# mistralai/mistral-inference

Hardware: NVIDIA H100
Metric: decode tokens/sec (bf16, batch=1, seq=4k) [+ prefill TFLOPS, both vs roofline] (higher is better)
Workload: dtype bf16

## Files before the change

include/mistral_b200.h:

```cpp
#ifndef MISTRAL_B200_H_
#define MISTRAL_B200_H_

#include <stddef.h>
#include <stdint.h>

#ifdef __cplusplus
extern "C" {
#endif

#define MB200_ABI_VERSION 1

#define MB200_OK 0
#define MB200_E_INVALID (-1)
#define MB200_E_WORKSPACE (-2)
#define MB200_E_CUDA (-3)

int mb200_abi_version(void);
const char* mb200_last_error(void);
int mb200_device_info(int* sm_count, int* max_smem_optin);

int mb200_rmsnorm(const void* x, const void* w, void* out, int64_t T, int64_t dim, float eps, void* stream);

int mb200_attn_qkv(const void* x, const void* norm_w, const void* wqkv, const float* rope, const int32_t* positions,
                   void* q_out, void* k_out, void* v_out, void* cache_k, void* cache_v, const int32_t* cache_rows,
// ... 26 lines not shown
int mb200_argmax_rows(const float* logits, int64_t* out_dev, int64_t T, int64_t vocab, void* stream);
int mb200_logprob_gather(const float* logits, const int64_t* target_dev, float* out_dev, int64_t T, int64_t vocab, void* stream);
int mb200_sample_top_p(const float* logits, const float* uniform_dev, int64_t* out_dev, int64_t T, int64_t vocab,
                       float temperature, float top_p, void* stream);

typedef struct mb200_moe_comm {
  int32_t n_ranks, my_rank;
  void* peer_yw[8];
  void* my_flags;
  void* peer_flags[8];
  void* epoch;
  void* done_counter;
} mb200_moe_comm;
int mb200_moe_sizes(int64_t T, int64_t n_experts, int64_t top_k, int64_t* tile_rows, int64_t* rows_cap, int64_t* plan_words);
int mb200_moe_route(const void* hn, const void* gate_w, int64_t T, int64_t dim, int64_t n_experts, int64_t top_k, int64_t shard_rank,
                    int64_t shard_world, int32_t* sel, void* wts, int32_t* slot, int32_t* plan, void* xs, void* row_w, void* stream);
int mb200_moe_grouped_ffn(const void* xs, const void* const* w13_host, const void* const* w2_host, const int32_t* plan, const void* row_w,
                          const int32_t* slot, const void* residual, void* g, void* yw, void* out, int64_t T, int64_t dim,
                          int64_t hidden, int64_t n_experts, int64_t top_k, const mb200_moe_comm* comm, void* workspace,
                          size_t workspace_bytes, void* stream);

int mb200_comm_alloc(size_t bytes, void** ptr_out);
int mb200_comm_free(void* ptr);
int mb200_comm_export(void* ptr, void* handle_out64);
int mb200_comm_open(const void* handle64, void** ptr_out);
int mb200_comm_close(void* ptr);

size_t mb200_workspace_bytes(int64_t T, int64_t dim, int64_t n_heads, int64_t n_kv_heads, int64_t head_dim,
                             int64_t hidden, int64_t vocab, int64_t max_batch);

typedef struct mb200_layer_desc {
  const void* wqkv;
  const void* wo;
  const void* w13;
  const void* w2;
  const void* attn_norm;
  const void* ffn_norm;
  void* cache_k;
  void* cache_v;
} mb200_layer_desc;

int mb200_decode_step(const mb200_layer_desc* layers_dev, const int32_t* windows_dev, int64_t n_layers, const void* emb,
                      const void* final_norm, const void* w_out, const float* rope, const int64_t* token_dev, int64_t pos,
                      int64_t batch_row, float* logits, int64_t* next_token_dev, int64_t dim, int64_t hidden, int64_t n_heads, int64_t n_kv_heads,
                      int64_t head_dim, int64_t vocab, float eps, int64_t n_experts, int64_t top_k, const void* const* moe_gate_dev,
                      const void* const* moe_w13_dev, const void* const* moe_w2_dev, void* workspace, size_t workspace_bytes, void* stream);

#define MB200_SKINNY_MAX_T 4

#define MB200_WORKSPACE_HEADER_BYTES (64 * 1024)

int mb200_debug_set_decode_timeline(void* device_buffer);
int mb200_debug_set_barrier_timeline(void* device_buffer);
int mb200_debug_launch_log(int enable, char* out, size_t out_bytes);

int mb200_test_gemm_naive(const void* a, const void* w, float* c, int64_t T, int64_t N, int64_t K, void* stream);

#ifdef __cplusplus
}
#endif
#endif
```

mistral_inference_b200/_abi.py:

```python
import ctypes
import os
from ctypes import c_char_p, c_float, c_int, c_int64, c_size_t, c_void_p
from pathlib import Path
from typing import Optional

import torch

_LIB_PATH = Path(os.environ.get("MB200_LIB_PATH") or Path(__file__).resolve().parent / "libmb200.so")
_lib: Optional[ctypes.CDLL] = None

ABI_VERSION = 1
SKINNY_MAX_T = 4
WORKSPACE_HEADER_BYTES = 64 * 1024

_SIGNATURES = {
    "mb200_abi_version": (c_int, []),
    "mb200_last_error": (c_char_p, []),
    "mb200_device_info": (c_int, [ctypes.POINTER(c_int), ctypes.POINTER(c_int)]),
    "mb200_rmsnorm": (c_int, [c_void_p, c_void_p, c_void_p, c_int64, c_int64, c_float, c_void_p]),
    "mb200_attn_qkv": (c_int, [c_void_p, c_void_p, c_void_p, c_void_p, c_void_p, c_void_p, c_void_p, c_void_p, c_void_p, c_void_p,
                               c_void_p, c_int64, c_int64, c_int64, c_int64, c_int64, c_float, c_void_p, c_size_t, c_void_p]),
    "mb200_kv_ring_write": (c_int, [c_void_p, c_void_p, c_void_p, c_void_p, c_void_p, c_int64, c_int64, c_int64, c_void_p]),
    "mb200_attn_decode": (c_int, [c_void_p, c_void_p, c_void_p, c_void_p, c_void_p, c_int64, c_int64, c_int64, c_int64, c_int64,
                                  c_int64, c_void_p, c_size_t, c_void_p]),
    "mb200_attn_prefill": (c_int, [c_void_p, c_void_p, c_void_p, c_void_p, c_void_p, c_void_p, c_void_p, c_void_p, c_int64, c_int64,
                                   c_int64, c_int64, c_int64, c_int64, c_int64, c_int, c_void_p]),
    "mb200_linear_residual": (c_int, [c_void_p, c_void_p, c_void_p, c_void_p, c_int64, c_int64, c_int64, c_void_p, c_size_t, c_void_p]),
    "mb200_ffn_gateup": (c_int, [c_void_p, c_void_p, c_void_p, c_void_p, c_int64, c_int64, c_int64, c_float, c_void_p, c_size_t,
                                 c_void_p]),
    "mb200_lm_head": (c_int, [c_void_p, c_void_p, c_void_p, c_void_p, c_int64, c_int64, c_int64, c_float, c_void_p, c_size_t,
                              c_void_p]),
    "mb200_decode_meta": (c_int, [c_void_p, c_void_p, c_int64, c_void_p, c_int64, c_void_p]),
    "mb200_argmax_rows": (c_int, [c_void_p, c_void_p, c_int64, c_int64, c_void_p]),
    "mb200_logprob_gather": (c_int, [c_void_p, c_void_p, c_void_p, c_int64, c_int64, c_void_p]),
    "mb200_sample_top_p": (c_int, [c_void_p, c_void_p, c_void_p, c_int64, c_int64, c_float, c_float, c_void_p]),
    "mb200_moe_sizes": (c_int, [c_int64, c_int64, c_int64, ctypes.POINTER(c_int64), ctypes.POINTER(c_int64), ctypes.POINTER(c_int64)]),
    "mb200_moe_route": (c_int, [c_void_p, c_void_p, c_int64, c_int64, c_int64, c_int64, c_int64, c_int64, c_void_p, c_void_p, c_void_p, c_void_p,
                                c_void_p, c_void_p, c_void_p]),
    "mb200_moe_grouped_ffn": (c_int, [c_void_p, c_void_p, c_void_p, c_void_p, c_void_p, c_void_p, c_void_p, c_void_p, c_void_p, c_void_p, c_int64,
                                      c_int64, c_int64, c_int64, c_int64, c_void_p, c_void_p, c_size_t, c_void_p]),
    "mb200_comm_alloc": (c_int, [c_size_t, ctypes.POINTER(c_void_p)]),
    "mb200_comm_free": (c_int, [c_void_p]),
    "mb200_comm_export": (c_int, [c_void_p, c_void_p]),
    "mb200_comm_open": (c_int, [c_void_p, ctypes.POINTER(c_void_p)]),
    "mb200_comm_close": (c_int, [c_void_p]),
    "mb200_workspace_bytes": (c_size_t, [c_int64] * 8),
    "mb200_decode_step": (c_int, [c_void_p, c_void_p, c_int64, c_void_p, c_void_p, c_void_p, c_void_p, c_void_p, c_int64, c_int64,
                                  c_void_p, c_void_p, c_int64, c_int64, c_int64, c_int64, c_int64, c_int64, c_float, c_int64, c_int64, c_void_p,
                                  c_void_p, c_void_p, c_void_p, c_size_t, c_void_p]),
    "mb200_debug_set_decode_timeline": (c_int, [c_void_p]),
    "mb200_debug_set_barrier_timeline": (c_int, [c_void_p]),
    "mb200_debug_launch_log": (c_int, [c_int, c_void_p, c_size_t]),
    "mb200_test_gemm_naive": (c_int, [c_void_p, c_void_p, c_void_p, c_int64, c_int64, c_int64, c_void_p]),
}


class Mb200Error(RuntimeError):
    pass


def library_path() -> Path:
    return _LIB_PATH


def lib() -> ctypes.CDLL:
    global _lib
    if _lib is not None:
        return _lib
    if not _LIB_PATH.exists():
        raise Mb200Error(
            f"{_LIB_PATH} not found: build it with `python -m mistral_inference_b200.build` "
            "(there is no PyTorch/CPU fallback for the hot path)")
    handle = ctypes.CDLL(str(_LIB_PATH), mode=os.RTLD_LOCAL if hasattr(os, "RTLD_LOCAL") else 0)
    for name, (restype, argtypes) in _SIGNATURES.items():
        fn = getattr(handle, name)
        fn.restype = restype
        fn.argtypes = argtypes
    if handle.mb200_abi_version() != ABI_VERSION:
        raise Mb200Error(f"libmb200 ABI {handle.mb200_abi_version()} != expected {ABI_VERSION}")
    _lib = handle
    return handle


def _check(rc: int, what: str) -> None:
    if rc != 0:
        msg = lib().mb200_last_error()
        raise Mb200Error(f"{what} failed ({rc}): {msg.decode() if msg else '?'}")


def _ptr(t: Optional[torch.Tensor]) -> Optional[int]:
    if t is None:
        return None
    assert t.is_cuda and t.is_contiguous(), "libmb200 takes contiguous CUDA tensors"
    return t.data_ptr()


def _stream() -> int:
    return torch.cuda.current_stream().cuda_stream


class Workspace:

    def __init__(self, nbytes: int, device: torch.device):
        self.buf = torch.zeros(max(int(nbytes), WORKSPACE_HEADER_BYTES + 256), dtype=torch.uint8, device=device)
# ... 148 lines not shown


def comm_alloc(nbytes: int) -> int:
    p = c_void_p(0)
    _check(lib().mb200_comm_alloc(nbytes, ctypes.byref(p)), "mb200_comm_alloc")
    return int(p.value)


def comm_free(ptr: int) -> None:
    _check(lib().mb200_comm_free(ptr), "mb200_comm_free")


def comm_export(ptr: int) -> bytes:
    h = ctypes.create_string_buffer(64)
    _check(lib().mb200_comm_export(ptr, ctypes.cast(h, c_void_p)), "mb200_comm_export")
    return h.raw


def comm_open(handle: bytes) -> int:
    h = ctypes.create_string_buffer(handle, 64)
    p = c_void_p(0)
    _check(lib().mb200_comm_open(ctypes.cast(h, c_void_p), ctypes.byref(p)), "mb200_comm_open")
    return int(p.value)


def comm_close(ptr: int) -> None:
    _check(lib().mb200_comm_close(ptr), "mb200_comm_close")


def decode_meta(seqpos_dev: torch.Tensor, meta_dev: torch.Tensor, windows) -> None:
    B = seqpos_dev.shape[0]
    arr = (ctypes.c_int32 * len(windows))(*[int(w) for w in windows])
    assert seqpos_dev.dtype == torch.int32 and meta_dev.dtype == torch.int32 and meta_dev.numel() >= 3 * B + 1 + 2 * B * len(windows)
    _check(lib().mb200_decode_meta(_ptr(seqpos_dev), _ptr(meta_dev), B, ctypes.cast(arr, c_void_p), len(windows), _stream()), "mb200_decode_meta")


def decode_step(layers_dev, windows_dev, n_layers, emb, final_norm, w_out, rope, token_dev, pos, batch_row, logits, next_token, dim, hidden,
                n_heads, n_kv_heads, head_dim, vocab, eps, ws: Workspace, n_experts: int = 0, top_k: int = 0, moe_gate=None, moe_w13=None,
                moe_w2=None) -> None:
    _check(lib().mb200_decode_step(_ptr(layers_dev), _ptr(windows_dev), n_layers, _ptr(emb), _ptr(final_norm), _ptr(w_out), _ptr(rope),
                                   _ptr(token_dev), pos, batch_row, _ptr(logits), _ptr(next_token), dim, hidden, n_heads, n_kv_heads, head_dim,
                                   vocab, eps, n_experts, top_k, _ptr(moe_gate), _ptr(moe_w13), _ptr(moe_w2), ws.ptr, ws.nbytes, _stream()),
           "mb200_decode_step")


def set_decode_timeline(buf: Optional[torch.Tensor]) -> None:
    _check(lib().mb200_debug_set_decode_timeline(_ptr(buf)), "mb200_debug_set_decode_timeline")


def set_barrier_timeline(buf: Optional[torch.Tensor]) -> None:
    _check(lib().mb200_debug_set_barrier_timeline(_ptr(buf)), "mb200_debug_set_barrier_timeline")


def launch_log(enable: bool) -> list:
    buf = ctypes.create_string_buffer(32768)
    _check(lib().mb200_debug_launch_log(int(enable), ctypes.cast(buf, c_void_p), len(buf)), "mb200_debug_launch_log")
    return buf.value.decode().splitlines()


def test_gemm_naive(a, w) -> torch.Tensor:
    T, K = a.shape
    c = torch.empty(T, w.shape[0], dtype=torch.float32, device=a.device)
    _check(lib().mb200_test_gemm_naive(_ptr(a), _ptr(w), _ptr(c), T, w.shape[0], K, _stream()), "mb200_test_gemm_naive")
    return c
```

mistral_inference_b200/csrc/abi.cu:

```cuda
#include <cmath>
#include <cstdlib>
#include <cstring>

#include "attn_decode.cuh"
#include "attn_decode_tma.cuh"
#include "attn_prefill.cuh"
#include "attn_prefill_wgmma.cuh"
#include "decode_megakernel.cuh"
#include "elementwise.cuh"
#include "gemm_mma.cuh"
#include "gemm_streamk.cuh"
#include "gemm_wgmma.cuh"
#include "moe.cuh"
#include "sampling.cuh"
#include "skinny_linear.cuh"

namespace mb200 {
thread_local char g_err[512] = "";
thread_local bool g_launch_log_on = false;
thread_local bool g_launch_log_overflow = false;
thread_local size_t g_launch_log_len = 0;
thread_local char g_launch_log[kLaunchLogBytes] = "";
static unsigned long long* g_mk_prof = nullptr;
static unsigned long long* g_mk_prof_bar = nullptr;

constexpr size_t kWsHeader = 64 * 1024;
inline size_t align256(size_t v) { return (v + 255) & ~(size_t)255; }

static int run_rmsnorm(const void* x, const void* w, void* out, int64_t T, int64_t dim, float eps, cudaStream_t st) {
  MB_CHECK_ARG(dim % 8 == 0 && T >= 0, "rmsnorm: dim=%lld must be a multiple of 8", (long long)dim);
  if (T == 0) return MB200_OK;
  MB_CHECK_CUDA(launch_pdl(rmsnorm_kernel, dim3((unsigned)T), dim3(256), 0, st, (const uint4*)x, (const uint4*)w, (uint4*)out, (int)dim, eps));
  return MB200_OK;
}

template <int MODE>
static int run_linear(const void* x, const void* norm_w, const void* w, const EpiParams& epi, int64_t T, int64_t N, int64_t K, float eps,
                      void* workspace, size_t workspace_bytes, cudaStream_t st) {
  MB_CHECK_ARG(T >= 1, "linear: T=%lld", (long long)T);
  if (T <= MB200_SKINNY_MAX_T) {
    SkinnyParams p;
    p.x = x;
    p.norm_w = norm_w;
    p.w = w;
    p.N = (int)N;
    p.K = (int)K;
    p.eps = eps;
    p.epi = epi;
    return norm_w ? launch_skinny<MODE, true>(p, (int)T, st) : launch_skinny<MODE, false>(p, (int)T, st);
  }
  const void* a = x;
  if (norm_w) {
    const size_t need = kWsHeader + SK_PARTIAL_BYTES + align256((size_t)T * K * 2);
    if (workspace == nullptr || workspace_bytes < need) return fail(MB200_E_WORKSPACE, "linear: workspace %zu < %zu", workspace_bytes, need);
    void* normed = (uint8_t*)workspace + kWsHeader + SK_PARTIAL_BYTES;
    int rc = run_rmsnorm(x, norm_w, normed, T, K, eps, st);
    if (rc) return rc;
    a = normed;
  }
  GemmParams g;
  g.a = a;
  g.w = w;
  g.T = (int)T;
  g.N = (int)N;
  g.K = (int)K;
  g.epi = epi;
  if (streamk_eligible(T, N, K)) return launch_streamk<MODE>(g, workspace, workspace_bytes, kWsHeader, st);
  if (wgmma_gemm_eligible(T, N, K)) return launch_gemm_wgmma<MODE>(g, st);
  return launch_gemm_mma<MODE>(g, st);
}
}

using namespace mb200;

extern "C" {

int mb200_abi_version(void) { return MB200_ABI_VERSION; }
// ... 383 lines not shown
  auto cut_ok = [](int64_t K) { const int64_t nch = (K + MK_MAX_KC - 1) / MK_MAX_KC; return K % (nch * 8) == 0; };
  MB_CHECK_ARG(n_kv_heads * kHeadDim * 2 + MK_KV_PAD <= MK_STAGE_BYTES / 8, "decode_step: a ring stage must hold 8 padded K/V position rows");
  MB_CHECK_ARG(cut_ok(dim) && cut_ok(hidden) && cut_ok(q_dim), "decode_step: dim/hidden/q_dim must split into 16-byte-aligned row chunks");
  MB_CHECK_ARG(vocab % 2 == 0 && hidden % 1 == 0, "decode_step: vocab must be even");
  int dev = 0, sms = 0, smem_max = 0, coop = 0;
  MB_CHECK_CUDA(cudaGetDevice(&dev));
  MB_CHECK_CUDA(cudaDeviceGetAttribute(&sms, cudaDevAttrMultiProcessorCount, dev));
  MB_CHECK_CUDA(cudaDeviceGetAttribute(&smem_max, cudaDevAttrMaxSharedMemoryPerBlockOptin, dev));
  MB_CHECK_CUDA(cudaDeviceGetAttribute(&coop, cudaDevAttrCooperativeLaunch, dev));
  MB_CHECK_ARG(coop, "decode_step: device does not support cooperative launch");

  MkParams p;
  p.layers = reinterpret_cast<const MkLayer*>(layers_dev);
  p.windows = windows_dev;
  p.n_layers = (int)n_layers;
  p.emb = (const bf16*)emb;
  p.final_norm = (const bf16*)final_norm;
  p.w_out = (const bf16*)w_out;
  p.rope = rope;
  p.token = token_dev;
  p.pos = (int)pos;
  p.batch_row = (int)batch_row;
  p.logits = logits;
  p.next_token = (long long*)next_token_dev;
  MB_CHECK_ARG(n_experts == 0 || (moe_gate_dev && moe_w13_dev && moe_w2_dev && top_k >= 1 && top_k <= MK_MAX_TOPK && top_k <= n_experts && n_experts <= 32),
               "decode_step: bad MoE arguments (E=%lld, k=%lld)", (long long)n_experts, (long long)top_k);
  p.n_experts = (int)n_experts;
  p.top_k = (int)(n_experts ? top_k : 0);
  p.moe_gate = (const bf16* const*)moe_gate_dev;
  p.moe_w13 = (const bf16* const*)moe_w13_dev;
  p.moe_w2 = (const bf16* const*)moe_w2_dev;
  p.dim = (int)dim;
  p.hidden = (int)hidden;
  p.H = (int)n_heads;
  p.KV = (int)n_kv_heads;
  p.vocab = (int)vocab;
  p.eps = eps;
  int64_t widest = dim > hidden ? dim : hidden;
  if (q_dim > widest) widest = q_dim;
  size_t xs_bytes = (size_t)widest * 2;
  if (n_experts && xs_bytes < (size_t)top_k * hidden * 2) xs_bytes = (size_t)top_k * hidden * 2;
  if (xs_bytes < 2048) xs_bytes = 2048;
  xs_bytes = (xs_bytes + 127) & ~(size_t)127;
  const size_t tail = 2 * MK_MAX_STAGES * sizeof(uint64_t) + 48 * sizeof(float) + sizeof(MoeRoute) + 8 + 64;
  int n_stages = (int)(((size_t)smem_max - xs_bytes - tail) / MK_STAGE_BYTES);
  if (n_stages > MK_MAX_STAGES) n_stages = MK_MAX_STAGES;
  MB_CHECK_ARG(n_stages > MK_CONSUMER_WARPS, "decode_step: not enough shared memory for the weight ring (%d stages)", n_stages);
  p.n_stages = n_stages;
  p.xs_bytes = (int)xs_bytes;
  {
    static int cap = -1;
    if (cap < 0) {
      const char* e = getenv("MB200_MK_INFLIGHT");
      cap = e ? atoi(e) : 5;
    }
    p.inflight_cap = cap < 2 ? 2 : (cap > 8 ? 8 : cap);
    static int kvu = -1;
    if (kvu < 0) {
      const char* e2 = getenv("MB200_MK_KV_UNCAPPED");
      kvu = e2 ? atoi(e2) : 0;
    }
    p.kv_uncapped = kvu;
  }
  const size_t smem = (size_t)n_stages * MK_STAGE_BYTES + xs_bytes + tail;

  MB_CHECK_ARG(n_kv_heads <= MK_CONSUMER_WARPS, "decode_step: n_kv_heads=%lld > %d (one consumer warp per kv head)", (long long)n_kv_heads,
               MK_CONSUMER_WARPS);
  uint8_t* ws = (uint8_t*)workspace;
  p.attn_counters = (int*)(ws + 8192);
  p.argmax_counter = (int*)(ws + 12288);
  p.argmax_slots = (unsigned long long*)(ws + 32768);
  p.bar_flags = (unsigned*)(ws + 16384);
  p.bar_epoch = (unsigned*)(ws + 20480);
  p.done_counter = (int*)(ws + 20480 + 128);
  size_t off = kWsHeader;
  auto take = [&](size_t bytes) { uint8_t* r = ws + off; off += align256(bytes); return r; };
  p.xbuf = (bf16*)take((size_t)2 * dim * 2);
  p.hbuf = (bf16*)take((size_t)dim * 2);
  p.qbuf = (bf16*)take((size_t)q_dim * 2);
  p.abuf = (bf16*)take((size_t)q_dim * 2);
  p.gbuf = (bf16*)take((size_t)(n_experts ? top_k : 1) * hidden * 2);
  p.partial = (float*)take((size_t)sms * n_heads * (kHeadDim + 2) * sizeof(float));
  p.prof = g_mk_prof;
  p.prof_bar = g_mk_prof_bar;
  if (workspace_bytes < off) return fail(MB200_E_WORKSPACE, "decode_step: workspace %zu < %zu", workspace_bytes, off);

  void* args[] = {(void*)&p};
  const void* fn = nullptr;
  switch (rep) {
    case 1: fn = (const void*)decode_megakernel<1>; break;
    case 2: fn = (const void*)decode_megakernel<2>; break;
    case 4: fn = (const void*)decode_megakernel<4>; break;
    case 6: fn = (const void*)decode_megakernel<6>; break;
    case 8: fn = (const void*)decode_megakernel<8>; break;
    default: return fail(MB200_E_INVALID, "decode_step: H/KV=%d unsupported (1,2,4,6,8)", rep);
  }
  MB_CHECK_CUDA(cudaFuncSetAttribute(fn, cudaFuncAttributeMaxDynamicSharedMemorySize, (int)smem));
  MB_CHECK_CUDA(cudaLaunchCooperativeKernel(fn, dim3((unsigned)sms), dim3(MK_THREADS), args, smem, (cudaStream_t)stream));
  return MB200_OK;
}

int mb200_debug_set_decode_timeline(void* device_buffer) {
  g_mk_prof = (unsigned long long*)device_buffer;
  return MB200_OK;
}
int mb200_debug_set_barrier_timeline(void* device_buffer) {
  g_mk_prof_bar = (unsigned long long*)device_buffer;
  return MB200_OK;
}

int mb200_debug_launch_log(int enable, char* out, size_t out_bytes) {
  const bool overflow = g_launch_log_overflow;
  const size_t len = g_launch_log_len;
  g_launch_log_on = enable != 0;
  g_launch_log_overflow = false;
  g_launch_log_len = 0;
  if (out != nullptr) {
    if (out_bytes < len + 1) return fail(MB200_E_INVALID, "launch log: %zu bytes recorded, buffer of %zu", len, out_bytes);
    memcpy(out, g_launch_log, len);
    out[len] = '\0';
  }
  if (overflow) return fail(MB200_E_INVALID, "launch log: more than %zu bytes of launches since the last read", kLaunchLogBytes);
  return MB200_OK;
}

int mb200_test_gemm_naive(const void* a, const void* w, float* c, int64_t T, int64_t N, int64_t K, void* stream) {
  MB_CHECK_ARG(a && w && c, "test_gemm_naive: null pointer");
  const dim3 grid((unsigned)ceil_div(N, 128), (unsigned)T);
  gemm_naive_kernel<<<grid, 128, 0, (cudaStream_t)stream>>>((const bf16*)a, (const bf16*)w, c, (int)T, (int)N, (int)K);
  MB_CHECK_LAUNCH("gemm_naive_kernel");
  return MB200_OK;
}

}

#ifdef MB200_SK_TRACE
extern "C" int mb200_debug_sk_trace(void* host_out, size_t bytes, unsigned* count) {
  using namespace mb200;
  if (bytes < sizeof(sk_trace_buf)) return fail(MB200_E_INVALID, "sk trace: %zu < %zu", bytes, sizeof(sk_trace_buf));
  MB_CHECK_CUDA(cudaDeviceSynchronize());
  MB_CHECK_CUDA(cudaMemcpyFromSymbol(host_out, sk_trace_buf, sizeof(sk_trace_buf)));
  MB_CHECK_CUDA(cudaMemcpyFromSymbol(count, sk_trace_count, sizeof(unsigned)));
  return MB200_OK;
}
#endif
```

mistral_inference_b200/csrc/decode_megakernel.cuh:

```cuda
#pragma once
#include "attn_decode.cuh"
#include "common.cuh"
#include "gemm_mma.cuh"

namespace mb200 {

constexpr int MK_CONSUMER_WARPS = 8;
constexpr int MK_CONSUMERS = MK_CONSUMER_WARPS * 32;
#ifndef MB200_MK_PRODUCERS
#define MB200_MK_PRODUCERS 2
#endif
constexpr int MK_PRODUCER_WARPS = MB200_MK_PRODUCERS;
#ifndef MB200_MK_WG
#define MB200_MK_WG 0
#endif
#if MB200_MK_WG
constexpr int MK_THREADS = MK_CONSUMERS + 128;
#else
constexpr int MK_THREADS = MK_CONSUMERS + 32 * MK_PRODUCER_WARPS;
#endif
constexpr int MK_WEIGHT_STAGE_BYTES = 16 * 1024;
constexpr int MK_MAX_KC = MK_WEIGHT_STAGE_BYTES / 4;
constexpr int MK_KV_PAD = 16;
constexpr int MK_STAGE_BYTES = 16 * 1024 + 16 * MK_KV_PAD;
constexpr int MK_MAX_STAGES = 12;
constexpr int MK_MAX_SPLITS = 32;

struct MkLayer {
  const bf16* wqkv;
  const bf16* wo;
  const bf16* w13;
  const bf16* w2;
  const bf16* attn_norm;
  const bf16* ffn_norm;
  bf16* cache_k;
  bf16* cache_v;
};

struct MkParams {
  const MkLayer* layers;
  const int32_t* windows;
  int n_experts, top_k;
  const bf16* const* moe_gate;
  const bf16* const* moe_w13;
  const bf16* const* moe_w2;
  int n_layers;
  const bf16* emb;
  const bf16* final_norm;
  const bf16* w_out;
  const float* rope;
  const int64_t* token;
  int pos;
  int batch_row;
  float* logits;
  long long* next_token;
  unsigned long long* argmax_slots;
  int* argmax_counter;
  int dim, hidden, H, KV, vocab;
  float eps;
  int n_stages, xs_bytes;
  int inflight_cap;
  int kv_uncapped;
  unsigned* bar_flags;
  unsigned* bar_epoch;
  int* done_counter;
  int* attn_counters;
  bf16* xbuf;
  bf16* hbuf;
  bf16* qbuf;
  bf16* abuf;
  bf16* gbuf;
  float* partial;
  unsigned long long* prof_bar;
  unsigned long long* prof;
};

__device__ __forceinline__ void mk_stamp(const MkParams& p, int tid, int layer, int idx) {
  if (p.prof != nullptr && tid == 0 && blockIdx.x % 21 == 0) {
    unsigned long long t;
    asm volatile("mov.u64 %0, %globaltimer;" : "=l"(t));
    p.prof[((blockIdx.x / 21) * p.n_layers + layer) * 16 + idx] = t;
  }
}

__device__ __forceinline__ uint32_t smem_u32(const void* p) { return (uint32_t)__cvta_generic_to_shared(p); }
__device__ __forceinline__ void mbar_init(uint64_t* bar, uint32_t count) {
  asm volatile("mbarrier.init.shared::cta.b64 [%0], %1;" ::"r"(smem_u32(bar)), "r"(count));
}
__device__ __forceinline__ void mbar_arrive(uint64_t* bar) {
  asm volatile("mbarrier.arrive.shared::cta.b64 _, [%0];" ::"r"(smem_u32(bar)) : "memory");
}
__device__ __forceinline__ void mbar_arrive_n(uint64_t* bar, uint32_t n) {
  asm volatile("mbarrier.arrive.shared::cta.b64 _, [%0], %1;" ::"r"(smem_u32(bar)), "r"(n) : "memory");
}
__device__ __forceinline__ void mbar_arrive_expect_tx(uint64_t* bar, uint32_t bytes) {
  asm volatile("mbarrier.arrive.expect_tx.shared::cta.b64 _, [%0], %1;" ::"r"(smem_u32(bar)), "r"(bytes) : "memory");
}
#ifndef MB200_WATCHDOG_SPINS
#define MB200_WATCHDOG_SPINS (1u << 22)
#endif
__device__ __forceinline__ bool mbar_try_wait(uint64_t* bar, uint32_t parity) {
  uint32_t ok;
  asm volatile(
      "{\n"
      ".reg .pred p;\n"
      "mbarrier.try_wait.parity.shared::cta.b64 p, [%1], %2;\n"
      "selp.u32 %0, 1, 0, p;\n"
      "}\n"
      : "=r"(ok)
      : "r"(smem_u32(bar)), "r"(parity)
      : "memory");
  return ok != 0;
}
__device__ __forceinline__ void mbar_wait(uint64_t* bar, uint32_t parity, int tag = 0, uint32_t it = 0) {
  uint32_t spins = 0;
  while (!mbar_try_wait(bar, parity)) {
    if (++spins == MB200_WATCHDOG_SPINS) {
      printf("[mb200 watchdog] block %d thread %d stuck in mbarrier wait tag=%d it=%u parity=%u\n", (int)blockIdx.x, (int)threadIdx.x, tag, it,
             parity);
      __trap();
    }
  }
}
__device__ __forceinline__ void mbar_wait_quiet(uint64_t* bar, uint32_t parity) {
  uint32_t spins = 0;
  while (!mbar_try_wait(bar, parity)) {
    if (++spins == MB200_WATCHDOG_SPINS) __trap();
  }
}
__device__ __forceinline__ void bulk_g2s(void* smem_dst, const void* gsrc, uint32_t bytes, uint64_t* bar) {
  asm volatile("cp.async.bulk.shared::cluster.global.mbarrier::complete_tx::bytes [%0], [%1], %2, [%3];" ::"r"(smem_u32(smem_dst)),
               "l"(gsrc), "r"(bytes), "r"(smem_u32(bar))
               : "memory");
}
// ... 50 lines not shown
  grid_arrive(p, tid, epoch, layer, which);
  grid_wait(p, tid, epoch, 0, MK_BAR_WORDS - 1);
  bar_stamp(p, tid, layer, which, 1);
}

struct MatCut {
  int pairs, nch, kc, p0, p1;
};
__device__ __forceinline__ MatCut cut_matrix(int N, int K) {
  MatCut c;
  c.pairs = N >> 1;
  c.nch = (K + MK_MAX_KC - 1) / MK_MAX_KC;
  c.kc = K / c.nch;
  c.p0 = (int)(((long long)blockIdx.x * c.pairs) / gridDim.x);
  c.p1 = (int)(((long long)(blockIdx.x + 1) * c.pairs) / gridDim.x);
  return c;
}

constexpr int MK_MAX_TOPK = 4;
struct MoeRoute {
  int e[MK_MAX_TOPK];
  float w[MK_MAX_TOPK];
};

struct RingState {
  uint32_t it;
};


constexpr float kMaskedScore = -1.0e30f;

struct AttnSlice {
  int C, k_begin, k_end, n_kvst, pps, n_slices;
};
__device__ __forceinline__ AttnSlice attn_slice(const MkParams& p, int W) {
  AttnSlice a;
  const int len = min(p.pos + 1, W);
  a.C = (len + (int)gridDim.x - 1) / (int)gridDim.x;
  a.n_slices = (len + a.C - 1) / a.C;
  a.k_begin = min((int)blockIdx.x * a.C, len);
  a.k_end = min(a.k_begin + a.C, len);
  a.pps = min(16, (MK_STAGE_BYTES / (p.KV * kHeadDim * 2 + MK_KV_PAD)) & ~7);
  a.n_kvst = (a.k_end - a.k_begin + a.pps - 1) / a.pps;
  return a;
}

__device__ __forceinline__ void bulk_g2s_hint(void* smem_dst, const void* gsrc, uint32_t bytes, uint64_t* bar, uint64_t policy) {
  asm volatile("cp.async.bulk.shared::cluster.global.mbarrier::complete_tx::bytes.L2::cache_hint [%0], [%1], %2, [%3], %4;" ::"r"(
                   smem_u32(smem_dst)),
               "l"(gsrc), "r"(bytes), "r"(smem_u32(bar)), "l"(policy)
               : "memory");
}

struct Producer {
  uint8_t* ring;
  uint64_t* full;
  uint64_t* empty;
  int n_stages;
  uint32_t it;
  uint64_t policy;

  int cap;
  int me, n_prod;
  bool kv_uncapped;
  uint32_t slot, par;
  uint32_t cslot, cpar;

  __device__ __forceinline__ void advance() {
    ++it;
    if (++slot == (uint32_t)n_stages) {
      slot = 0;
      par ^= 1;
    }
    if (it > (uint32_t)cap && ++cslot == (uint32_t)n_stages) {
      cslot = 0;
      cpar ^= 1;
    }
  }
  __device__ __forceinline__ uint8_t* acquire(uint32_t bytes, uint64_t*& bar, bool capped = true) {
    if ((int)(it % (uint32_t)n_prod) != me) {
      advance();
      return nullptr;
    }
    if (capped && it >= (uint32_t)cap) mbar_wait(&full[cslot], cpar, 7, it);
    mbar_wait(&empty[slot], par ^ 1, 1, it);
    bar = &full[slot];
    mbar_arrive_expect_tx(bar, bytes);
    uint8_t* dst = ring + (size_t)slot * MK_STAGE_BYTES;
    advance();
    return dst;
  }

  __device__ __forceinline__ void matrix(const bf16* W, int N, int K) {
    const MatCut c = cut_matrix(N, K);
    const uint32_t row_bytes = (uint32_t)c.kc * 2;
    for (int g0 = c.p0; g0 < c.p1; g0 += MK_CONSUMER_WARPS) {
      const int g = min(MK_CONSUMER_WARPS, c.p1 - g0);
      for (int ch = 0; ch < c.nch; ++ch) {
        for (int w = 0; w < g; ++w) {
          const bf16* r0 = W + (int64_t)(2 * (g0 + w)) * K;
          uint64_t* bar;
          uint8_t* dst = acquire(2 * row_bytes, bar);
          if (dst == nullptr) continue;
          if (c.nch == 1) {
            bulk_g2s_hint(dst, r0, 2 * row_bytes, bar, policy);
          } else {
            bulk_g2s_hint(dst, r0 + ch * c.kc, row_bytes, bar, policy);
            bulk_g2s_hint(dst + row_bytes, r0 + K + ch * c.kc, row_bytes, bar, policy);
          }
        }
      }
    }
  }

  __device__ __forceinline__ void moe_down(const bf16* const* w2, const int* sel, int top_k, int N, int K) {
    const MatCut c = cut_matrix(N, K);
    const uint32_t row_bytes = (uint32_t)c.kc * 2;
    for (int g0 = c.p0; g0 < c.p1; g0 += MK_CONSUMER_WARPS) {
      const int g = min(MK_CONSUMER_WARPS, c.p1 - g0);
      for (int j = 0; j < top_k; ++j) {
        const bf16* W = w2[sel[j]];
        for (int ch = 0; ch < c.nch; ++ch) {
          for (int w = 0; w < g; ++w) {
            const bf16* r0 = W + (int64_t)(2 * (g0 + w)) * K;
            uint64_t* bar;
            uint8_t* dst = acquire(2 * row_bytes, bar);
            if (dst == nullptr) continue;
            if (c.nch == 1) {
              bulk_g2s_hint(dst, r0, 2 * row_bytes, bar, policy);
            } else {
              bulk_g2s_hint(dst, r0 + ch * c.kc, row_bytes, bar, policy);
              bulk_g2s_hint(dst + row_bytes, r0 + K + ch * c.kc, row_bytes, bar, policy);
            }
          }
        }
      }
    }
  }

  __device__ __forceinline__ void kv_slice(const MkParams& p, const MkLayer& L, int W) {
    const AttnSlice a = attn_slice(p, W);
    const int64_t row_elems = (int64_t)p.KV * kHeadDim;
    const uint32_t row_bytes = (uint32_t)row_elems * 2;
    const bf16* kbase = L.cache_k + ((int64_t)p.batch_row * W) * row_elems;
    const bf16* vbase = L.cache_v + ((int64_t)p.batch_row * W) * row_elems;
    for (int j = 0; j < a.n_kvst; ++j) {
      const int k0 = a.k_begin + j * a.pps;
      const int rows = min(a.pps, a.k_end - k0);
#pragma unroll
      for (int kv = 0; kv < 2; ++kv) {
        uint64_t* bar;
        uint8_t* dst = acquire((uint32_t)rows * row_bytes, bar, !kv_uncapped);
        if (dst == nullptr) continue;
        const bf16* src = (kv ? vbase : kbase) + (int64_t)k0 * row_elems;
        for (int r = 0; r < rows; ++r) bulk_g2s_hint(dst + r * (row_bytes + MK_KV_PAD), src + (int64_t)r * row_elems, row_bytes, bar, policy);
      }
    }
  }
};

__device__ __forceinline__ void producer_main(const MkParams& p, uint8_t* ring, uint64_t* full, uint64_t* empty, int me, const MoeRoute* route,
                                              uint64_t* route_bar) {
  Producer pr;
  pr.ring = ring;
  pr.full = full;
  pr.empty = empty;
  pr.n_stages = p.n_stages;
  pr.it = 0;
  pr.cap = p.inflight_cap;
  pr.me = me;
  pr.n_prod = MK_PRODUCER_WARPS;
  pr.kv_uncapped = p.kv_uncapped != 0;
  pr.slot = pr.par = pr.cslot = pr.cpar = 0;
  asm volatile("createpolicy.fractional.L2::evict_first.b64 %0, 1.0;" : "=l"(pr.policy));
  const int q_dim = p.H * kHeadDim, kv_dim = p.KV * kHeadDim;
  for (int l = 0; l < p.n_layers; ++l) {
    const MkLayer L = p.layers[l];
    pr.matrix(L.wqkv, q_dim + 2 * kv_dim, p.dim);
    pr.kv_slice(p, L, p.windows[l]);
    pr.matrix(L.wo, p.dim, q_dim);
    if (p.n_experts == 0) {
      pr.matrix(L.w13, 2 * p.hidden, p.dim);
      pr.matrix(L.w2, p.dim, p.hidden);
    } else {
      mbar_wait(route_bar, (uint32_t)(l & 1), 8, (uint32_t)l);
      int sel[MK_MAX_TOPK];
      for (int j = 0; j < p.top_k; ++j) sel[j] = route->e[j];
      for (int j = 0; j < p.top_k; ++j) pr.matrix(p.moe_w13[l * p.n_experts + sel[j]], 2 * p.hidden, p.dim);
      pr.moe_down(p.moe_w2 + l * p.n_experts, sel, p.top_k, p.dim, p.hidden);
    }
  }
  pr.matrix(p.w_out, p.vocab, p.dim);
}

template <class Ready, class Pre, class Epi>
__device__ __forceinline__ void consume_matrix(int N, int K, const uint8_t* ring, uint64_t* full, uint64_t* empty, int n_stages, RingState& rs,
                                               const uint4* xs, int tid, Ready ready, Pre pre, Epi epi) {
  const MatCut c = cut_matrix(N, K);
  const int lane = tid & 31, warp = tid >> 5;
  const int kc8 = c.kc >> 3;
  for (int g0 = c.p0; g0 < c.p1; g0 += MK_CONSUMER_WARPS) {
    const int g = min(MK_CONSUMER_WARPS, c.p1 - g0);
    float a0 = 0.f, a1 = 0.f;
    uint2 prefetched = make_uint2(0u, 0u);
    if (warp < g && lane == 0) prefetched = pre(2 * (g0 + warp));
    for (int ch = 0; ch < c.nch; ++ch) {
      if (g0 == c.p0) ready(ch);
      if (warp < g) {
        const uint32_t it = rs.it + (uint32_t)(ch * g + warp);
        const uint32_t slot = it % n_stages, par = (it / n_stages) & 1;
        mbar_wait(&empty[slot], par ^ 1, 2, it);
        mbar_wait(&full[slot], par, 3, it);
        const uint4* w0 = reinterpret_cast<const uint4*>(ring + (size_t)slot * MK_STAGE_BYTES);
        const uint4* w1 = w0 + kc8;
        const uint4* xc = xs + ch * kc8;
#pragma unroll 4
        for (int i = lane; i < kc8; i += 32) {
          const uint4 a = w0[i], b = w1[i], x = xc[i];
          const uint32_t aw[4] = {a.x, a.y, a.z, a.w}, bw[4] = {b.x, b.y, b.z, b.w}, xw[4] = {x.x, x.y, x.z, x.w};
#pragma unroll
          for (int j = 0; j < 4; ++j) {
            const float xl = bf16lo(xw[j]), xh = bf16hi(xw[j]);
            a0 = fmaf(bf16lo(aw[j]), xl, a0);
            a0 = fmaf(bf16hi(aw[j]), xh, a0);
            a1 = fmaf(bf16lo(bw[j]), xl, a1);
            a1 = fmaf(bf16hi(bw[j]), xh, a1);
          }
        }
        __syncwarp();
        if (lane == 0) mbar_arrive_n(&empty[slot], MK_CONSUMER_WARPS);
      }
    }
    if (warp < g) {
      a0 = warp_sum(a0);
      a1 = warp_sum(a1);
      if (lane == 0) epi(2 * (g0 + warp), a0, a1, prefetched);
    }
    rs.it += (uint32_t)(g * c.nch);
    consumer_sync();
  }
}

__device__ __forceinline__ void stage_x(uint4* xs, const bf16* src, const bf16* norm_w, int K, float eps, float* red, int tid) {
  const int kc = K >> 3;
// ... 318 lines not shown
            const uint32_t aw[4] = {a.x, a.y, a.z, a.w}, bw[4] = {b.x, b.y, b.z, b.w}, xw[4] = {x.x, x.y, x.z, x.w};
#pragma unroll
            for (int q = 0; q < 4; ++q) {
              const float xl = bf16lo(xw[q]), xh = bf16hi(xw[q]);
              a0 = fmaf(bf16lo(aw[q]), xl, a0);
              a0 = fmaf(bf16hi(aw[q]), xh, a0);
              a1 = fmaf(bf16lo(bw[q]), xl, a1);
              a1 = fmaf(bf16hi(bw[q]), xh, a1);
            }
          }
          __syncwarp();
          if (lane == 0) mbar_arrive_n(&empty[slot], MK_CONSUMER_WARPS);
        }
        a0 = warp_sum(a0);
        a1 = warp_sum(a1);
        const float t0 = round_bf16(rt.w[j] * round_bf16(a0)), t1 = round_bf16(rt.w[j] * round_bf16(a1));
        r0 = (j == 0) ? t0 : round_bf16(r0 + t0);
        r1 = (j == 0) ? t1 : round_bf16(r1 + t1);
      }
      if (lane == 0) epi(2 * (g0 + warp), r0, r1, prefetched);
    }
    rs.it += (uint32_t)(g * c.nch * p.top_k);
    consumer_sync();
  }
}

template <int REP>
__global__ void __launch_bounds__(MK_THREADS, 1) decode_megakernel(const MkParams p) {
  extern __shared__ __align__(128) uint8_t smem[];
  uint8_t* ring = smem;
  uint4* xs = reinterpret_cast<uint4*>(smem + (size_t)p.n_stages * MK_STAGE_BYTES);
  uint64_t* full = reinterpret_cast<uint64_t*>(reinterpret_cast<uint8_t*>(xs) + p.xs_bytes);
  uint64_t* empty = full + MK_MAX_STAGES;
  float* red = reinterpret_cast<float*>(empty + MK_MAX_STAGES);
  MoeRoute* route = reinterpret_cast<MoeRoute*>(red + 48);
  uint64_t* route_bar = reinterpret_cast<uint64_t*>(route + 1);

  const int tid = threadIdx.x;
  if (tid == 0) {
    for (int i = 0; i < p.n_stages; ++i) {
      mbar_init(&full[i], 1);
      mbar_init(&empty[i], MK_CONSUMER_WARPS);
    }
    mbar_init(route_bar, 1);
    asm volatile("fence.mbarrier_init.release.cluster;" ::: "memory");
  }
  __syncthreads();

  const int q_dim = p.H * kHeadDim, kv_dim = p.KV * kHeadDim;
  RingState rs;
  rs.it = 0;

  if (tid >= MK_CONSUMERS) {
#if MB200_MK_WG
    asm volatile("setmaxnreg.dec.sync.aligned.u32 120;");
    if ((tid & 31) == 0 && ((tid - MK_CONSUMERS) >> 5) < MK_PRODUCER_WARPS)
#else
    if ((tid & 31) == 0)
#endif
      producer_main(p, ring, full, empty, (tid - MK_CONSUMERS) >> 5, route, route_bar);
    return;
  }
#if MB200_MK_WG
  asm volatile("setmaxnreg.inc.sync.aligned.u32 192;");
#endif

  unsigned epoch = ld_acquire_u32(p.bar_epoch);
  const unsigned epoch0 = epoch;
  const int64_t token = *p.token;
  for (int l = 0; l < p.n_layers; ++l) {
    const MkLayer L = p.layers[l];
    const int W = p.windows[l];
    const bf16* x_in = (l == 0) ? p.emb + token * p.dim : p.xbuf + (size_t)(l & 1) * p.dim;
    bf16* x_out = p.xbuf + (size_t)((l + 1) & 1) * p.dim;

    mk_stamp(p, tid, l, 0);
    stage_x(xs, x_in, L.attn_norm, p.dim, p.eps, red, tid);
    mk_stamp(p, tid, l, 1);
    {
      const int slot_row = p.batch_row * W + p.pos % W;
      const float* rope_row = p.rope + (int64_t)p.pos * (kHeadDim / 2) * 2;
      bf16* ck = L.cache_k + (int64_t)slot_row * kv_dim;
      bf16* cv = L.cache_v + (int64_t)slot_row * kv_dim;
      consume_matrix(q_dim + 2 * kv_dim, p.dim, ring, full, empty, p.n_stages, rs, xs, tid, [&](int) {},
                     [&](int n) { return *reinterpret_cast<const uint2*>(rope_row + ((n & (kHeadDim - 1)) >> 1) * 2); },
                     [&](int n, float a0, float a1, uint2 pf) {
        const float y0 = round_bf16(a0), y1 = round_bf16(a1);
        if (n < q_dim + kv_dim) {
          const float2 cs = make_float2(__uint_as_float(pf.x), __uint_as_float(pf.y));
          float re, im;
          ref_cmul(y0, y1, cs.x, cs.y, re, im);
          const uint32_t packed = pack_bf16x2(re, im);
          if (n < q_dim)
            *reinterpret_cast<uint32_t*>(p.qbuf + n) = packed;
          else
            *reinterpret_cast<uint32_t*>(ck + (n - q_dim)) = packed;
        } else {
          *reinterpret_cast<uint32_t*>(cv + (n - q_dim - kv_dim)) = pack_bf16x2(y0, y1);
        }
      });
    }
    mk_stamp(p, tid, l, 2);
    grid_barrier(p, tid, epoch, l, 0);
    mk_stamp(p, tid, l, 3);

    if (attn_slice(p, W).pps == 16)
      mk_attention_slice<REP, 16>(p, L, W, ring, full, empty, p.n_stages, rs, tid, l);
    else
      mk_attention_slice<REP, 8>(p, L, W, ring, full, empty, p.n_stages, rs, tid, l);
    mk_stamp(p, tid, l, 12);
    grid_barrier(p, tid, epoch, l, 1);
    mk_stamp(p, tid, l, 13);
    mk_attention_combine(p, W, tid, reinterpret_cast<float*>(xs));
    mk_stamp(p, tid, l, 4);
    grid_barrier(p, tid, epoch, l, 2);
    mk_stamp(p, tid, l, 5);

    stage_x(xs, p.abuf, nullptr, q_dim, 0.f, red, tid);
// ... 99 lines not shown
```

Measured before the change: 167.0.

## Prefetch upcoming weight rows into L2 while producers wait, lower inflight cap

Producer warps in the decode megakernel now issue cp.async.bulk L2 prefetches up to 128KB ahead inside the current matrix while they wait for a ring slot to free. The default inflight cap drops from 5 to 2, since L2 run-ahead is meant to keep HBM busy without deep shared-memory staging. The KV-uncapped option and the warpgroup register-reallocation variant are removed, and optional per-segment producer stall counters are added for profiling. The change risks duplicated or wasted L2 traffic and a shallower pipeline if the prefetch does not hide latency.

```diff
diff --git a/include/mistral_b200.h b/include/mistral_b200.h
--- a/include/mistral_b200.h
+++ b/include/mistral_b200.h
@@ -102,6 +102,7 @@
 
 int mb200_debug_set_decode_timeline(void* device_buffer);
 int mb200_debug_set_barrier_timeline(void* device_buffer);
+int mb200_debug_set_producer_stalls(void* device_buffer);
 int mb200_debug_launch_log(int enable, char* out, size_t out_bytes);
 
 int mb200_test_gemm_naive(const void* a, const void* w, float* c, int64_t T, int64_t N, int64_t K, void* stream);
diff --git a/mistral_inference_b200/_abi.py b/mistral_inference_b200/_abi.py
--- a/mistral_inference_b200/_abi.py
+++ b/mistral_inference_b200/_abi.py
@@ -50,6 +50,7 @@
                                   c_void_p, c_void_p, c_void_p, c_size_t, c_void_p]),
     "mb200_debug_set_decode_timeline": (c_int, [c_void_p]),
     "mb200_debug_set_barrier_timeline": (c_int, [c_void_p]),
+    "mb200_debug_set_producer_stalls": (c_int, [c_void_p]),
     "mb200_debug_launch_log": (c_int, [c_int, c_void_p, c_size_t]),
     "mb200_test_gemm_naive": (c_int, [c_void_p, c_void_p, c_void_p, c_int64, c_int64, c_int64, c_void_p]),
 }
@@ -304,6 +305,10 @@
     _check(lib().mb200_debug_set_barrier_timeline(_ptr(buf)), "mb200_debug_set_barrier_timeline")
 
 
+def set_producer_stalls(buf: Optional[torch.Tensor]) -> None:
+    _check(lib().mb200_debug_set_producer_stalls(_ptr(buf)), "mb200_debug_set_producer_stalls")
+
+
 def launch_log(enable: bool) -> list:
     buf = ctypes.create_string_buffer(32768)
     _check(lib().mb200_debug_launch_log(int(enable), ctypes.cast(buf, c_void_p), len(buf)), "mb200_debug_launch_log")
diff --git a/mistral_inference_b200/csrc/abi.cu b/mistral_inference_b200/csrc/abi.cu
--- a/mistral_inference_b200/csrc/abi.cu
+++ b/mistral_inference_b200/csrc/abi.cu
@@ -23,6 +23,7 @@
 thread_local char g_launch_log[kLaunchLogBytes] = "";
 static unsigned long long* g_mk_prof = nullptr;
 static unsigned long long* g_mk_prof_bar = nullptr;
+static unsigned long long* g_mk_stall = nullptr;
 
 constexpr size_t kWsHeader = 64 * 1024;
 inline size_t align256(size_t v) { return (v + 255) & ~(size_t)255; }
@@ -512,15 +513,9 @@
     static int cap = -1;
     if (cap < 0) {
       const char* e = getenv("MB200_MK_INFLIGHT");
-      cap = e ? atoi(e) : 5;
+      cap = e ? atoi(e) : 2;
     }
     p.inflight_cap = cap < 2 ? 2 : (cap > 8 ? 8 : cap);
-    static int kvu = -1;
-    if (kvu < 0) {
-      const char* e2 = getenv("MB200_MK_KV_UNCAPPED");
-      kvu = e2 ? atoi(e2) : 0;
-    }
-    p.kv_uncapped = kvu;
   }
   const size_t smem = (size_t)n_stages * MK_STAGE_BYTES + xs_bytes + tail;
 
@@ -543,6 +538,7 @@
   p.partial = (float*)take((size_t)sms * n_heads * (kHeadDim + 2) * sizeof(float));
   p.prof = g_mk_prof;
   p.prof_bar = g_mk_prof_bar;
+  p.stall = g_mk_stall;
   if (workspace_bytes < off) return fail(MB200_E_WORKSPACE, "decode_step: workspace %zu < %zu", workspace_bytes, off);
 
   void* args[] = {(void*)&p};
@@ -566,6 +562,10 @@
 }
 int mb200_debug_set_barrier_timeline(void* device_buffer) {
   g_mk_prof_bar = (unsigned long long*)device_buffer;
+  return MB200_OK;
+}
+int mb200_debug_set_producer_stalls(void* device_buffer) {
+  g_mk_stall = (unsigned long long*)device_buffer;
   return MB200_OK;
 }
 
diff --git a/mistral_inference_b200/csrc/decode_megakernel.cuh b/mistral_inference_b200/csrc/decode_megakernel.cuh
--- a/mistral_inference_b200/csrc/decode_megakernel.cuh
+++ b/mistral_inference_b200/csrc/decode_megakernel.cuh
@@ -11,19 +11,17 @@
 #define MB200_MK_PRODUCERS 2
 #endif
 constexpr int MK_PRODUCER_WARPS = MB200_MK_PRODUCERS;
-#ifndef MB200_MK_WG
-#define MB200_MK_WG 0
-#endif
-#if MB200_MK_WG
-constexpr int MK_THREADS = MK_CONSUMERS + 128;
-#else
 constexpr int MK_THREADS = MK_CONSUMERS + 32 * MK_PRODUCER_WARPS;
-#endif
 constexpr int MK_WEIGHT_STAGE_BYTES = 16 * 1024;
 constexpr int MK_MAX_KC = MK_WEIGHT_STAGE_BYTES / 4;
 constexpr int MK_KV_PAD = 16;
 constexpr int MK_STAGE_BYTES = 16 * 1024 + 16 * MK_KV_PAD;
 constexpr int MK_MAX_STAGES = 12;
+#ifndef MB200_MK_L2_AHEAD
+#define MB200_MK_L2_AHEAD (128 * 1024)
+#endif
+constexpr int64_t MK_L2_AHEAD = MB200_MK_L2_AHEAD;
+enum MkSegment { MK_SEG_QKV, MK_SEG_KV, MK_SEG_WO, MK_SEG_W13, MK_SEG_W2, MK_SEG_LM_HEAD, MK_SEGMENTS };
 constexpr int MK_MAX_SPLITS = 32;
 
 struct MkLayer {
@@ -60,7 +58,6 @@
   float eps;
   int n_stages, xs_bytes;
   int inflight_cap;
-  int kv_uncapped;
   unsigned* bar_flags;
   unsigned* bar_epoch;
   int* done_counter;
@@ -73,13 +70,17 @@
   float* partial;
   unsigned long long* prof_bar;
   unsigned long long* prof;
+  unsigned long long* stall;
 };
 
+__device__ __forceinline__ int mk_sample_stride() { return ((int)gridDim.x + 7) / 8; }
 __device__ __forceinline__ void mk_stamp(const MkParams& p, int tid, int layer, int idx) {
-  if (p.prof != nullptr && tid == 0 && blockIdx.x % 21 == 0) {
+  if (p.prof != nullptr && tid == 0) {
+    const int stride = mk_sample_stride();
+    if (blockIdx.x % stride != 0) return;
     unsigned long long t;
     asm volatile("mov.u64 %0, %globaltimer;" : "=l"(t));
-    p.prof[((blockIdx.x / 21) * p.n_layers + layer) * 16 + idx] = t;
+    p.prof[((blockIdx.x / stride) * p.n_layers + layer) * 16 + idx] = t;
   }
 }
 
@@ -236,6 +237,15 @@
                : "memory");
 }
 
+__device__ __noinline__ void mk_wait_counted(uint64_t* bar, uint32_t parity, int tag, uint32_t it, unsigned long long* ctr) {
+  if (mbar_try_wait(bar, parity)) return;
+  unsigned long long t0, t1;
+  asm volatile("mov.u64 %0, %globaltimer;" : "=l"(t0));
+  mbar_wait(bar, parity, tag, it);
+  asm volatile("mov.u64 %0, %globaltimer;" : "=l"(t1));
+  atomicAdd(ctr, t1 - t0);
+}
+
 struct Producer {
   uint8_t* ring;
   uint64_t* full;
@@ -246,9 +256,17 @@
 
   int cap;
   int me, n_prod;
-  bool kv_uncapped;
   uint32_t slot, par;
   uint32_t cslot, cpar;
+  unsigned long long* stall;
+  int seg;
+
+  __device__ __forceinline__ void wait(uint64_t* bar, uint32_t parity, int tag, int kind) {
+    if (stall == nullptr)
+      mbar_wait(bar, parity, tag, it);
+    else
+      mk_wait_counted(bar, parity, tag, it, stall + seg * 2 + kind);
+  }
 
   __device__ __forceinline__ void advance() {
     ++it;
@@ -261,13 +279,24 @@
       cpar ^= 1;
     }
   }
-  __device__ __forceinline__ uint8_t* acquire(uint32_t bytes, uint64_t*& bar, bool capped = true) {
+  const uint8_t* pf;
+  __device__ __forceinline__ void run_ahead(const uint8_t* ahead, const uint8_t* ahead_end) {
+    if (pf < ahead || pf > ahead + MK_L2_AHEAD) pf = ahead;
+    const uint8_t* lim = ahead + MK_L2_AHEAD < ahead_end ? ahead + MK_L2_AHEAD : ahead_end;
+    while (pf < lim && !mbar_try_wait(&empty[slot], par ^ 1)) {
+      const uint32_t n = (uint32_t)min((int64_t)MK_WEIGHT_STAGE_BYTES, (int64_t)(lim - pf));
+      asm volatile("cp.async.bulk.prefetch.L2.global [%0], %1;" ::"l"(pf), "r"(n) : "memory");
+      pf += n;
+    }
+  }
+  __device__ __forceinline__ uint8_t* acquire(uint32_t bytes, uint64_t*& bar, const uint8_t* ahead = nullptr, const uint8_t* ahead_end = nullptr) {
     if ((int)(it % (uint32_t)n_prod) != me) {
       advance();
       return nullptr;
     }
-    if (capped && it >= (uint32_t)cap) mbar_wait(&full[cslot], cpar, 7, it);
-    mbar_wait(&empty[slot], par ^ 1, 1, it);
+    if (it >= (uint32_t)cap) wait(&full[cslot], cpar, 7, 1);
+    if (MK_L2_AHEAD > 0 && ahead != nullptr) run_ahead(ahead, ahead_end);
+    wait(&empty[slot], par ^ 1, 1, 0);
     bar = &full[slot];
     mbar_arrive_expect_tx(bar, bytes);
     uint8_t* dst = ring + (size_t)slot * MK_STAGE_BYTES;
@@ -284,7 +313,9 @@
         for (int w = 0; w < g; ++w) {
           const bf16* r0 = W + (int64_t)(2 * (g0 + w)) * K;
           uint64_t* bar;
-          uint8_t* dst = acquire(2 * row_bytes, bar);
+          uint8_t* dst = c.nch == 1 ? acquire(2 * row_bytes, bar, reinterpret_cast<const uint8_t*>(r0 + 2 * K),
+                                              reinterpret_cast<const uint8_t*>(W + (int64_t)(2 * c.p1) * K))
+                                    : acquire(2 * row_bytes, bar);
           if (dst == nullptr) continue;
           if (c.nch == 1) {
             bulk_g2s_hint(dst, r0, 2 * row_bytes, bar, policy);
@@ -334,7 +365,7 @@
 #pragma unroll
       for (int kv = 0; kv < 2; ++kv) {
         uint64_t* bar;
-        uint8_t* dst = acquire((uint32_t)rows * row_bytes, bar, !kv_uncapped);
+        uint8_t* dst = acquire((uint32_t)rows * row_bytes, bar);
         if (dst == nullptr) continue;
         const bf16* src = (kv ? vbase : kbase) + (int64_t)k0 * row_elems;
         for (int r = 0; r < rows; ++r) bulk_g2s_hint(dst + r * (row_bytes + MK_KV_PAD), src + (int64_t)r * row_elems, row_bytes, bar, policy);
@@ -354,26 +385,34 @@
   pr.cap = p.inflight_cap;
   pr.me = me;
   pr.n_prod = MK_PRODUCER_WARPS;
-  pr.kv_uncapped = p.kv_uncapped != 0;
   pr.slot = pr.par = pr.cslot = pr.cpar = 0;
+  pr.pf = nullptr;
+  pr.stall = p.stall != nullptr ? p.stall + (size_t)blockIdx.x * MK_SEGMENTS * 2 : nullptr;
   asm volatile("createpolicy.fractional.L2::evict_first.b64 %0, 1.0;" : "=l"(pr.policy));
   const int q_dim = p.H * kHeadDim, kv_dim = p.KV * kHeadDim;
   for (int l = 0; l < p.n_layers; ++l) {
     const MkLayer L = p.layers[l];
+    pr.seg = MK_SEG_QKV;
     pr.matrix(L.wqkv, q_dim + 2 * kv_dim, p.dim);
+    pr.seg = MK_SEG_KV;
     pr.kv_slice(p, L, p.windows[l]);
+    pr.seg = MK_SEG_WO;
     pr.matrix(L.wo, p.dim, q_dim);
+    pr.seg = MK_SEG_W13;
     if (p.n_experts == 0) {
       pr.matrix(L.w13, 2 * p.hidden, p.dim);
+      pr.seg = MK_SEG_W2;
       pr.matrix(L.w2, p.dim, p.hidden);
     } else {
       mbar_wait(route_bar, (uint32_t)(l & 1), 8, (uint32_t)l);
       int sel[MK_MAX_TOPK];
       for (int j = 0; j < p.top_k; ++j) sel[j] = route->e[j];
       for (int j = 0; j < p.top_k; ++j) pr.matrix(p.moe_w13[l * p.n_experts + sel[j]], 2 * p.hidden, p.dim);
+      pr.seg = MK_SEG_W2;
       pr.moe_down(p.moe_w2 + l * p.n_experts, sel, p.top_k, p.dim, p.hidden);
     }
   }
+  pr.seg = MK_SEG_LM_HEAD;
   pr.matrix(p.w_out, p.vocab, p.dim);
 }
 
@@ -798,18 +837,10 @@
   rs.it = 0;
 
   if (tid >= MK_CONSUMERS) {
-#if MB200_MK_WG
-    asm volatile("setmaxnreg.dec.sync.aligned.u32 120;");
-    if ((tid & 31) == 0 && ((tid - MK_CONSUMERS) >> 5) < MK_PRODUCER_WARPS)
-#else
     if ((tid & 31) == 0)
-#endif
       producer_main(p, ring, full, empty, (tid - MK_CONSUMERS) >> 5, route, route_bar);
     return;
   }
-#if MB200_MK_WG
-  asm volatile("setmaxnreg.inc.sync.aligned.u32 192;");
-#endif
 
   unsigned epoch = ld_acquire_u32(p.bar_epoch);
   const unsigned epoch0 = epoch;
```

Result: faster. 176.4 (median of 6 runs) (+5.7%).
